# pjhusky/vulkan-compute-tests

Measured on AMD Instinct MI355X. Metric: path-traced samples/s, higher is better.
Workload: dtype f32

## Files before the change

vulkan-compute-tests_amd/csrc/mc_math.h:

```cpp
#pragma once
#include <hip/hip_runtime.h>

namespace mc {
namespace dm {

__device__ __forceinline__ float as_float(uint32_t u) { return __uint_as_float(u); }
__device__ __forceinline__ uint32_t as_uint(float f) { return __float_as_uint(f); }

__device__ __forceinline__ float ieee_div(float a, float b) { return a / b; }
__device__ __forceinline__ float ieee_sqrt(float a) { return __builtin_sqrtf(a); }

__device__ __forceinline__ bool in_short_window(float x) { return (as_uint(x) - 0x0D800000u) < 0x64000000u; }
__device__ __forceinline__ bool wave_all(bool p) { return __builtin_amdgcn_ballot_w64(!p) == 0ull; }
__device__ __forceinline__ float sqrt_short(float x) {
    float y = __builtin_amdgcn_rsqf(x);
    float g = x * y;
    float d = __builtin_fmaf(-g, g, x);
    return __builtin_fmaf(d, 0.5f * y, g);
}
__device__ __forceinline__ float rcp_short(float b) {
    float r = __builtin_amdgcn_rcpf(b);
    float e = __builtin_fmaf(-b, r, 1.0f);
    return __builtin_fmaf(e, r, r);
}

__device__ __forceinline__ float rsqrt_short(float x) {
    const float y = __builtin_amdgcn_rsqf(x);
    const float g = x * y;
    const float d = __builtin_fmaf(-g, g, x);
    const float s = __builtin_fmaf(d, 0.5f * y, g);
    const float e = __builtin_fmaf(-s, y, 1.0f);
    const float r = __builtin_fmaf(e, y, y);
    const uint32_t tie = ((as_uint(x) & 0x00fffffeu) == 0x007ffffeu) ? 1u : 0u;
    return as_float(as_uint(r) + tie);
}

__device__ __forceinline__ float div_step(float a, float s, float y) {
    const float q0 = a * y;
    const float r = __builtin_fmaf(-s, q0, a);
    return __builtin_fmaf(r, y, q0);
}

template <int Fast> __device__ __forceinline__ float fdiv(float a, float b) {
    if (Fast == 2) return div_step(a, b, rcp_short(b));
    if (Fast) return a * __builtin_amdgcn_rcpf(b);
    return ieee_div(a, b);
}
template <int Fast, bool HaveY> __device__ __forceinline__ void div3(float& a0, float& a1, float& a2, float s, float y) {
    if constexpr (!Fast) {
        const uint32_t b0 = as_uint(a0), b1 = as_uint(a1), b2 = as_uint(a2);
        uint32_t hi = b0 > b1 ? b0 : b1; hi = hi > b2 ? hi : b2;
        const uint32_t l0 = b0 - 1u, l1 = b1 - 1u, l2 = b2 - 1u;
        uint32_t lo = l0 < l1 ? l0 : l1; lo = lo < l2 ? lo : l2;
        const bool outside = ((as_uint(s) - 0x21800000u) >= 0x3C000000u) | (hi >= 0x5D800000u) | (lo < 0x21800000u - 1u);
        if constexpr (!HaveY) y = rcp_short(s);
        const float q0 = div_step(a0, s, y), q1 = div_step(a1, s, y), q2 = div_step(a2, s, y);
        if (__builtin_expect(outside, 0)) { a0 = ieee_div(a0, s); a1 = ieee_div(a1, s); a2 = ieee_div(a2, s); }
        else { a0 = q0; a1 = q1; a2 = q2; }
        return;
    }
    a0 = fdiv<Fast>(a0, s); a1 = fdiv<Fast>(a1, s); a2 = fdiv<Fast>(a2, s);
}
template <int Fast> __device__ __forceinline__ float fsqrt(float a) {
    if (Fast == 2) { const float r = sqrt_short(a); return a == 0.0f ? 0.0f : r; }
    if (Fast) return __builtin_amdgcn_sqrtf(a);
    if (__builtin_expect(wave_all(in_short_window(a)), 1)) return sqrt_short(a);
    return ieee_sqrt(a);
}
template <int Fast> __device__ __forceinline__ float inversesqrt(float a) {
    if (Fast == 2) return rsqrt_short(a);
    if (Fast) return __builtin_amdgcn_rsqf(a);
    if (__builtin_expect(wave_all(in_short_window(a)), 1)) return rsqrt_short(a);
    return ieee_div(1.0f, ieee_sqrt(a));
}

__device__ __forceinline__ void sincos_reduce(float x, float& r, int& k) {
    const float TWO_OVER_PI = 0.636619772367581343f;
    const float PIO2_HI = 1.5703125f;
    const float PIO2_MID = 4.837512969970703125e-4f;
    const float PIO2_LO = 7.54978995489188216e-8f;
    float q = __builtin_rintf(x * TWO_OVER_PI);
    r = __builtin_fmaf(q, -PIO2_HI, x);
    r = __builtin_fmaf(q, -PIO2_MID, r);
    r = __builtin_fmaf(q, -PIO2_LO, r);
    k = (int)q;
}
__device__ __forceinline__ float sin_kernel(float r) {
    float z = r * r;
    float p = __builtin_fmaf(-1.9515295891e-4f, z, 8.3321608736e-3f);
    p = __builtin_fmaf(p, z, -1.6666654611e-1f);
    return __builtin_fmaf(p * z, r, r);
}
__device__ __forceinline__ float cos_kernel(float r) {
    float z = r * r;
    float p = __builtin_fmaf(2.443315711809948e-5f, z, -1.388731625493765e-3f);
    p = __builtin_fmaf(p, z, 4.166664568298827e-2f);
    float t = __builtin_fmaf(-0.5f, z, 1.0f);
    return __builtin_fmaf(p * z, z, t);
}
__device__ __forceinline__ float mc_sin(float x) {
    float r; int k; sincos_reduce(x, r, k);
    float s = (k & 1) ? cos_kernel(r) : sin_kernel(r);
    return (k & 2) ? -s : s;
}
__device__ __forceinline__ float mc_cos(float x) {
    float r; int k; sincos_reduce(x, r, k);
    float c = (k & 1) ? sin_kernel(r) : cos_kernel(r);
    return ((k + 1) & 2) ? -c : c;
}
__device__ __forceinline__ void mc_sincos(float x, float& s, float& c) {
    float r; int k; sincos_reduce(x, r, k);
    float sk = sin_kernel(r), ck = cos_kernel(r);
    float sv = (k & 1) ? ck : sk;
    float cv = (k & 1) ? sk : ck;
    s = as_float(as_uint(sv) ^ (((uint32_t)k << 30) & 0x80000000u));
    c = as_float(as_uint(cv) ^ (((uint32_t)(k + 1) << 30) & 0x80000000u));
}

template <int Fast> __device__ __forceinline__ void sincos_angle(float angle, float u, float& s, float& c) {
    if (Fast) {
        s = __builtin_amdgcn_sinf(u);
        c = __builtin_amdgcn_cosf(u);
    } else {
        mc_sincos(angle, s, c);
    }
}

#ifdef MC_PT_TRANS_UNGROUPED
constexpr bool kTransGroups = false;
#else
constexpr bool kTransGroups = true;
#endif
__device__ __forceinline__ void light_trans_group(float xcc, float u, float& inv_len, float& s, float& c) {
    inv_len = xcc;
    asm volatile("s_setprio 3\n\t"
                 "v_rsq_f32_e32 %0, %0\n\t"
                 "v_sin_f32_e32 %1, %3\n\t"
                 "v_cos_f32_e32 %2, %3\n\t"
                 "s_setprio 0\n\t"
                 "s_nop 0"
                 : "+v"(inv_len), "=&v"(s), "=&v"(c) : "v"(u));
}
__device__ __forceinline__ void bounce_trans_group(float u1, float u2, float& r2s, float& s1, float& c1, float& C) {
    C = 1.0f - u2;
    asm volatile("s_setprio 3\n\t"
                 "v_sqrt_f32_e32 %0, %5\n\t"
                 "v_sin_f32_e32 %1, %4\n\t"
                 "v_cos_f32_e32 %2, %4\n\t"
                 "v_sqrt_f32_e32 %3, %3\n\t"
                 "s_setprio 0\n\t"
                 "s_nop 0"
                 : "=&v"(r2s), "=&v"(s1), "=&v"(c1), "+v"(C) : "v"(u1), "v"(u2));
}

__device__ __forceinline__ float mc_log2(float x) {
    if (x == 0.0f) return -__builtin_inff();
    int e_adj = 0;
    if (x < 1.17549435e-38f) { x = x * 16777216.0f; e_adj = -24; }
    uint32_t u = as_uint(x);
    int e = (int)(u >> 23) - 127;
// ... 44 lines not shown
```

vulkan-compute-tests_amd/csrc/pathtrace_kernel.h:

```cpp
#pragma once
#include <hip/hip_runtime.h>

#include <cstdlib>
#include <type_traits>
#include <utility>

#include "mc_internal.h"
#include "ds_arith.h"
#include "mc_math.h"

namespace mc {
namespace pt {

constexpr int kMaxPlanes = 16;
constexpr int kMaxSpheres = 16;
constexpr int kMaxSlabSpheres = 8;

struct v3 {
    float x, y, z;
};

struct SceneArgs {
    uint32_t n_planes, n_spheres;
    uint32_t emissive_mask;
    uint32_t nee_skip_planes;
    uint32_t materials_known;
    uint32_t emit_skip_ok;
    uint32_t box_ok;
    float obj[(kMaxPlanes + kMaxSpheres) * 12];
    float r2[kMaxSpheres];
    float slab_w_pos[3], slab_w_neg[3];
    int32_t slab_id_pos[3], slab_id_neg[3];
    const float* d_obj;
    const float* d_obj_derived;
    const uint32_t* d_emissive;
    uint32_t n_emissive;
    uint32_t spheres_disjoint;
    uint32_t pad3, pad4;
};

struct PTArgs {
    uint32_t W, H, spp, sample_begin, sample_end, max_depth, row_begin, row_end, row_block, row_stride;
    v3 cam_o, cam_d, cx, cy, lc;
    float cam_oc[kMaxSlabSpheres][3], cam_occ[kMaxSlabSpheres];
    float inv_W, inv_H, inv_spp;
    float4* __restrict__ out;
    uint32_t* status;
    SceneArgs scene;
};

__device__ __forceinline__ v3 operator+(v3 a, v3 b) { return v3{a.x + b.x, a.y + b.y, a.z + b.z}; }
__device__ __forceinline__ v3 operator-(v3 a, v3 b) { return v3{a.x - b.x, a.y - b.y, a.z - b.z}; }
__device__ __forceinline__ v3 operator*(v3 a, v3 b) { return v3{a.x * b.x, a.y * b.y, a.z * b.z}; }
__device__ __forceinline__ v3 operator*(v3 a, float s) { return v3{a.x * s, a.y * s, a.z * s}; }
__device__ __forceinline__ v3 operator-(v3 a) { return v3{-a.x, -a.y, -a.z}; }
__device__ __forceinline__ float dot(v3 a, v3 b) { return (a.x * b.x + a.y * b.y) + a.z * b.z; }
__device__ __forceinline__ v3 cross(v3 a, v3 b) {
    return v3{a.y * b.z - b.y * a.z, a.z * b.x - b.z * a.x, a.x * b.y - b.x * a.y};
}
template <int Fast> __device__ __forceinline__ v3 normalize(v3 a) { return a * dm::inversesqrt<Fast>(dot(a, a)); }
template <int Fast, bool HaveY> __device__ __forceinline__ v3 divs_impl(v3 a, float s, float y) {
    dm::div3<Fast, HaveY>(a.x, a.y, a.z, s, y);
    return a;
}
template <int Fast> __device__ __forceinline__ v3 divs(v3 a, float s) { return divs_impl<Fast, false>(a, s, 0.0f); }
template <int Fast> __device__ __forceinline__ v3 divs_recip(v3 a, float s, float y) { return divs_impl<Fast, true>(a, s, y); }
template <int Fast> __device__ __forceinline__ v3 tangent_u(v3 w) {
    const bool sel = __builtin_fabsf(w.x) > 0.1f;
    if constexpr (Fast) {
        const float q = sel ? w.x : w.y;
        const float inv = dm::inversesqrt<Fast>(__builtin_fmaf(q, q, w.z * w.z));
        const float zi = w.z * inv, qi = q * inv;
        return v3{sel ? zi : 0.0f, sel ? 0.0f : -zi, sel ? -qi : qi};
    } else {
        return normalize<false>(cross(sel ? v3{0, 1, 0} : v3{1, 0, 0}, w));
    }
}
template <int Fast, bool UnitBasis> __device__ __forceinline__ v3 normalize_unit_combination(v3 a) {
    if constexpr (Fast == 1 && UnitBasis) return a;
    else return normalize<Fast>(a);
}
__device__ __forceinline__ v3 reflect(v3 I, v3 N) { return I - N * (2.0f * dot(N, I)); }
__device__ __forceinline__ v3 select(bool c, v3 a, v3 b) { return v3{c ? a.x : b.x, c ? a.y : b.y, c ? a.z : b.z}; }
__device__ __forceinline__ float comp(v3 a, int axis) { return axis == 0 ? a.x : (axis == 1 ? a.y : a.z); }

__device__ __forceinline__ v3 rand01(uint32_t x, uint32_t y, uint32_t z) {
#pragma unroll
    for (int i = 0; i < 3; i++) {
        uint32_t nx = ((x >> 8) ^ y) * 1103515245u;
        uint32_t ny = ((y >> 8) ^ z) * 1103515245u;
        uint32_t nz = ((z >> 8) ^ x) * 1103515245u;
        x = nx; y = ny; z = nz;
    }
    const float s = 2.3283064365386963e-10f;
    return v3{(float)x * s, (float)y * s, (float)z * s};
}

#ifdef MC_PT_REGION_STATS
static __device__ unsigned long long g_region_exec[32];
static __device__ unsigned long long g_region_lanes[32];
#define MC_REGION(r)                                                                            \
    do {                                                                                        \
        unsigned long long m_ = __ballot(1);                                                    \
        if ((int)__lane_id() == __ffsll((long long)m_) - 1) {                                   \
            atomicAdd(&g_region_exec[r], 1ull);                                                 \
            atomicAdd(&g_region_lanes[r], (unsigned long long)__popcll(m_));                    \
        }                                                                                       \
    } while (0)
#define MC_PT_REGION_STATS_READER(name)                                                                              \
    int name(unsigned long long* exec32, unsigned long long* lanes32) {                                              \
        unsigned long long e[32], l[32], zero[32] = {0};                                                             \
        if (hipMemcpyFromSymbol(e, HIP_SYMBOL(mc::pt::g_region_exec), sizeof(zero)) != hipSuccess) return 3;         \
        if (hipMemcpyFromSymbol(l, HIP_SYMBOL(mc::pt::g_region_lanes), sizeof(zero)) != hipSuccess) return 3;        \
        if (hipMemcpyToSymbol(HIP_SYMBOL(mc::pt::g_region_exec), zero, sizeof(zero)) != hipSuccess) return 3;        \
        if (hipMemcpyToSymbol(HIP_SYMBOL(mc::pt::g_region_lanes), zero, sizeof(zero)) != hipSuccess) return 3;       \
        for (int i = 0; i < 32; i++) { exec32[i] += e[i]; lanes32[i] += l[i]; }                                      \
        return 0;                                                                                                    \
    }
#else
#define MC_REGION(r) do { } while (0)
#define MC_PT_REGION_STATS_READER(name)
#endif

#ifndef MC_PT_DECISION_FP
#define MC_PT_DECISION_FP
#endif

constexpr float kEps = 1e-4f, kTriEps = 1e-7f, kInf = 1e20f;
constexpr float kPi = 3.141592653589793f;
constexpr float kInvPi = 1.0f / kPi;
static_assert(kInvPi == 0x1.45f306p-2f, "1/pi must be the correctly rounded fp32 quotient (numpy: float32(1)/float32(pi) = 0x3ea2f983)");

__device__ __forceinline__ bool needs_precision(const float* sp, v3 o) {
    const float maxLen = 500.0f;
    v3 c{sp[0], sp[1], sp[2]};
    v3 co = c - o;
    return sp[3] > maxLen || dot(c, c) > maxLen * maxLen || dot(o, o) > maxLen * maxLen || dot(co, co) > maxLen * maxLen;
}
template <int Fast, int Prec>
__device__ __forceinline__ bool sphere_extended(const float* sp, float r2, v3 o, v3 d, float& dd) {
    auto rsq = [](float x) { return dm::inversesqrt<Fast>(x); };
    if (Prec == 1) {
        double ocx = (double)sp[0] - (double)o.x, ocy = (double)sp[1] - (double)o.y, ocz = (double)sp[2] - (double)o.z;
        double dx = d.x, dy = d.y, dz = d.z;
        double b = (ocx * dx + ocy * dy) + ocz * dz;
        double det = (b * b - ((ocx * ocx + ocy * ocy) + ocz * ocz)) + (double)r2;
        if (det < 0) return false;
        det = __builtin_sqrt(det);
        dd = (float)(b - det);
        if (!(dd > kEps)) { dd = (float)(b + det); if (!(dd > kEps)) dd = kInf; }
        return true;
    } else if (Prec == 2) {
        ds2 ocX = ds_add(ds_set(sp[0]), ds_set(-o.x)), ocY = ds_add(ds_set(sp[1]), ds_set(-o.y)), ocZ = ds_add(ds_set(sp[2]), ds_set(-o.z));
        ds2 rdX = ds_set(d.x), rdY = ds_set(d.y), rdZ = ds_set(d.z);
        ds2 b = ds_dot3(ocX, ocY, ocZ, rdX, rdY, rdZ);
        ds2 w = ds_set(sp[3]);
        ds2 det = ds_add(ds_sub(ds_mul(b, b), ds_dot3(ocX, ocY, ocZ, ocX, ocY, ocZ)), ds_mul(w, w));
        if (ds_compare(det, ds_set(0.0f)) < 0.0f) return false;
        det = ds_sqrt(det, rsq);
        ds2 eps_ds = ds_set(kEps);
        ds2 bMinus = ds_sub(b, det), bPlus = ds_add(b, det);
        ds2 d_ds = bMinus;
        dd = d_ds.hi;
        if (ds_compare(d_ds, eps_ds) <= 0.0f) {
            d_ds = bPlus;
            dd = d_ds.hi;
            if (ds_compare(d_ds, eps_ds) <= 0.0f) dd = kInf;
        }
        return true;
    } else {
        ds2 ocX = df64_add(df64_from_f32(sp[0]), df64_from_f32(-o.x)), ocY = df64_add(df64_from_f32(sp[1]), df64_from_f32(-o.y)),
            ocZ = df64_add(df64_from_f32(sp[2]), df64_from_f32(-o.z));
        ds2 rdX = df64_from_f32(d.x), rdY = df64_from_f32(d.y), rdZ = df64_from_f32(d.z);
        ds2 b = df64_dot3(ocX, ocY, ocZ, rdX, rdY, rdZ);
        ds2 w = df64_from_f32(sp[3]);
        ds2 det = df64_add(df64_add(df64_mult(b, b), df64_mult(df64_dot3(ocX, ocY, ocZ, ocX, ocY, ocZ), df64_from_f32(-1.0f))),
                           df64_mult(w, w));
        if (df64_lt(det, df64_from_f32(0.0f))) return false;
        det = df64_sqrt(det, rsq);
        float bMinus = df64_add(b, df64_mult(det, df64_from_f32(-1.0f))).hi;
        float bPlus = df64_add(b, det).hi;
        dd = bMinus;
        if (!(dd > kEps)) { dd = bPlus; if (!(dd > kEps)) dd = kInf; }
        return true;
    }
}

__device__ __forceinline__ float to_vgpr(float uniform) {
    float v;
    asm volatile("v_mov_b32 %0, %1" : "=v"(v) : "s"(uniform));
    return v;
}
template <int NS> struct HotSlabN {
    static constexpr int ns = NS;
    float W_pos[3], W_negm[3];
    float c[NS][3], r2[NS];
    float eps, tri_eps, inf;
    template <bool InVgpr = true, bool WPosInVgpr = false> __device__ __forceinline__ void load(const SceneArgs& sc) {
        auto put = [](float u) { return InVgpr ? to_vgpr(u) : u; };
#pragma unroll
        for (int a = 0; a < 3; a++) { W_pos[a] = (InVgpr || WPosInVgpr) ? to_vgpr(sc.slab_w_pos[a]) : sc.slab_w_pos[a]; W_negm[a] = put(-sc.slab_w_neg[a]); }
#pragma unroll
        for (int i = 0; i < NS; i++) {
#pragma unroll
            for (int k = 0; k < 3; k++) c[i][k] = put(sc.obj[12 * (6 + i) + k]);
            r2[i] = put(sc.r2[i]);
        }
        eps = put(1e-4f); tri_eps = put(1e-7f); inf = put(1e20f);
    }
};

template <int Fast, bool Closed, bool OccR2, int StatsBase, bool HaveOc, int NS>
__device__ __forceinline__ int intersect_slab_impl(const HotSlabN<NS>& h, v3 o, v3 d, float& t_out, bool shadow_skip_planes,
                                                   const float* occ,
                                                   const v3* oc_at_o) {
    MC_PT_DECISION_FP
    static_assert(HaveOc || !OccR2, "the r^2-reduced squared lengths come from the caller");
    float t = h.inf;
    int id = -1;
    if (Fast && !shadow_skip_planes) {
        float num[3], den[3];
#pragma unroll
        for (int a = 0; a < 3; a++) {
            const float da = comp(d, a), oa = comp(o, a);
            const bool pos = da > 0.0f;
            num[a] = (pos ? h.W_pos[a] : h.W_negm[a]) - oa; den[a] = da;
        }
        float bn = num[0], bd = den[0];
        int bid = 1;
#pragma unroll
        for (int a = 1; a < 3; a++) {
            const bool nearer = __builtin_fabsf(num[a]) * __builtin_fabsf(bd) < __builtin_fabsf(bn) * __builtin_fabsf(den[a]);
            bn = nearer ? num[a] : bn; bd = nearer ? den[a] : bd; bid = nearer ? 2 * a + 1 : bid;
        }
        bid ^= (int)(dm::as_uint(bd) >> 31);
        const float dd = dm::fdiv<Fast>(bn, bd);
        if constexpr (Closed) { t = dd; id = bid; }
        else if (__builtin_fabsf(bd) > h.tri_eps && dd < t) { t = dd; id = bid; }
    } else if (!shadow_skip_planes) {
#pragma unroll
        for (int a = 0; a < 3; a++) {
            const float da = comp(d, a), oa = comp(o, a);
            const bool pos = da > 0.0f;
            const float W = pos ? h.W_pos[a] : h.W_negm[a];
            const float dd = dm::fdiv<Fast>(W - oa, da);
            if (__builtin_fabsf(da) > h.tri_eps && dd < t) { t = dd; id = pos ? 2 * a + 1 : 2 * a; }
        }
    }
#pragma unroll
    for (int i = 0; i < NS; i++) {
        v3 oc;
        if constexpr (HaveOc) oc = oc_at_o[i]; else oc = v3{h.c[i][0], h.c[i][1], h.c[i][2]} - o;
        float b = dot(oc, d);
        float occ_i;
        if constexpr (HaveOc) occ_i = occ[i]; else occ_i = dot(oc, oc);
        float det = OccR2 ? b * b - occ_i : (b * b - occ_i) + h.r2[i];
        if (!(det < 0.0f)) {
            if constexpr (StatsBase >= 0) MC_REGION(StatsBase + i);
            float sq = dm::fsqrt<Fast>(det);
            float dd = b - sq;
            if (dd <= h.eps) {
                dd = b + sq;
                if (dd <= h.eps) dd = h.inf;
            }
            if (dd < t) { t = dd; id = 6 + i; }
        }
    }
    t_out = t;
    if constexpr (Closed) return id;
    return (t < h.inf) ? id : -1;
}
template <int Fast, bool Closed = false, bool OccR2 = false, int StatsBase = -1, int NS = 3>
__device__ __forceinline__ int intersect_slab(const HotSlabN<NS>& h, v3 o, v3 d, float& t_out, bool shadow_skip_planes) {
    return intersect_slab_impl<Fast, Closed, OccR2, StatsBase, false, NS>(h, o, d, t_out, shadow_skip_planes, nullptr, nullptr);
}
template <int Fast, bool Closed = false, bool OccR2 = false, int StatsBase = -1, int NS = 3>
__device__ __forceinline__ int intersect_slab(const HotSlabN<NS>& h, v3 o, v3 d, float& t_out, bool shadow_skip_planes,
                                              const float* occ, const v3* oc_at_o) {
    return intersect_slab_impl<Fast, Closed, OccR2, StatsBase, true, NS>(h, o, d, t_out, shadow_skip_planes, occ, oc_at_o);
}

template <int Fast, bool OccR2 = false, int NS = 3>
__device__ __forceinline__ bool shadow_reaches_sphere(const HotSlabN<NS>& h, v3 o, v3 d, int li, v3 oc_li, const float* occ) {
    MC_PT_DECISION_FP
    float dd[NS];
#pragma unroll
    for (int i = 0; i < NS; i++) {
        const v3 oc = i == li ? oc_li : v3{h.c[i][0], h.c[i][1], h.c[i][2]} - o;
        float b = dot(oc, d);
        float det = OccR2 ? b * b - occ[i] : (b * b - occ[i]) + h.r2[i];
        float r = h.inf;
        if (!(det < 0.0f)) {
            float sq = dm::fsqrt<Fast>(det);
            r = b - sq;
            if (r <= h.eps) {
                r = b + sq;
                if (r <= h.eps) r = h.inf;
            }
        }
        dd[i] = r;
    }
    bool nearest = true;
#pragma unroll
    for (int k = 0; k < NS; k++) {
        if (k < li) nearest = nearest && dd[li] < dd[k];
        else if (k > li) nearest = nearest && !(dd[k] < dd[li]);
    }
    if (Fast && li == NS - 1 && NS > 1) return nearest;
    return nearest && dd[li] < h.inf;
}

template <bool OccR2, int NS>
__device__ __forceinline__ bool shadow_visible_disjoint(const HotSlabN<NS>& h, v3 d, int li, const v3* xoc, const float* occ) {
    MC_PT_DECISION_FP
    float b[NS];
    bool hit[NS];
#pragma unroll
    for (int i = 0; i < NS; i++) {
        b[i] = dot(xoc[i], d);
        const float det = OccR2 ? b[i] * b[i] - occ[i] : (b[i] * b[i] - occ[i]) + h.r2[i];
        if (i == li) { hit[i] = det >= 0.0f; continue; }
        const float e = b[i] - h.eps;
        hit[i] = !(det < 0.0f) && (e > 0.0f || det > e * e);
    }
    bool vis = hit[li];
#pragma unroll
    for (int i = 0; i < NS; i++)
        if (i != li) vis = vis && !(hit[i] && b[i] < b[li]);
    return vis;
}


template <int Fast, int NP, int NS, bool Slab, int Prec>
__device__ __forceinline__ int intersect(const SceneArgs& sc, const float* __restrict__ obj, v3 o, v3 d, float& t_out,
                                         bool shadow_skip_planes = false) {
    MC_PT_DECISION_FP
    constexpr bool LdsScene = NP < 0;
    const int np = NP >= 0 ? NP : (int)sc.n_planes;
    const int ns = NS >= 0 ? NS : (int)sc.n_spheres;
    float t = kInf;
    int id = -1;
    if (Slab && shadow_skip_planes) {
    } else if (Slab) {
#pragma unroll
        for (int a = 0; a < 3; a++) {
            const float da = comp(d, a), oa = comp(o, a);
            const bool pos = da > 0.0f;
            const float den = __builtin_fabsf(da);
            const float num = pos ? (sc.slab_w_pos[a] - oa) : (sc.slab_w_neg[a] + oa);
            const float dd = dm::fdiv<Fast>(num, den);
            if (den > kTriEps && dd < t) { t = dd; id = pos ? 2 * a + 1 : 2 * a; }
        }
    } else {
#pragma unroll
// ... 483 lines not shown
```

vulkan-compute-tests_amd/csrc/pathtrace_pool.h:

```cpp
#pragma once
#include <type_traits>
#include "pathtrace_kernel.h"

namespace mc {
namespace pt {

#ifdef MC_PT_POOL_PARENT_FORMS
constexpr bool kPoolParentForms = true;
#else
constexpr bool kPoolParentForms = false;
#endif
#if defined(MC_PT_POOL_FLOAT_STATE) || defined(MC_PT_POOL_PARENT_FORMS)
constexpr bool kPoolFloatState = true;
#else
constexpr bool kPoolFloatState = false;
#endif
__device__ __forceinline__ unsigned long long lanes_where(bool cmp) { return __builtin_amdgcn_ballot_w64(cmp); }
__device__ __forceinline__ bool lane_in(unsigned long long m) { return __builtin_amdgcn_inverse_ballot_w64(m); }
__device__ __forceinline__ v3 add_emission(v3 rad, v3 accmat, v3 e) {
#pragma clang fp contract(off)
    const float px = accmat.x * e.x, py = accmat.y * e.y, pz = accmat.z * e.z;
    return v3{rad.x + px, rad.y + py, rad.z + pz};
}
constexpr uint32_t kPoolEntryFloats = 8;
constexpr uint32_t kPoolRecordStride = 16;
template <int NS> constexpr uint32_t pool_record_floats() { return (6u + (uint32_t)NS) * kPoolRecordStride; }
constexpr uint32_t kPoolStashFloats = 128u * kPoolEntryFloats;
template <int NS> constexpr uint32_t pool_result_batches() { return NS <= 3 ? 3u : 4u; }
template <int NS> constexpr uint32_t pool_result_floats() { return 64u * pool_result_batches<NS>() * 3u; }
template <int Fast, int NS> constexpr uint32_t pool_wave_lds_floats() { return kPoolStashFloats + (Fast ? 0u : pool_result_floats<NS>()); }
template <int Fast, int NS> constexpr size_t pool_block_lds_bytes() { return (pool_record_floats<NS>() + 4u * pool_wave_lds_floats<Fast, NS>()) * sizeof(float); }
template <int Fast, int NS> constexpr int pool_waves() {
    constexpr int kFast3 = 7;
    constexpr int kStrict3 = 6;
    return Fast ? (NS <= 3 ? kFast3 : NS <= 5 ? 6 : NS <= 6 ? 5 : 4) : (NS <= 3 ? kStrict3 : NS <= 6 ? 4 : 3);
}

template <int Fast, int NS> constexpr bool pool_parent_state() { return kPoolFloatState || (Fast == 1 && NS == 2); }
template <int Fast, int NS> constexpr bool pool_lane_masks() { return !pool_parent_state<Fast, NS>() && Fast != 0 && !(Fast == 2 && NS == 7); }
template <int Fast, int NS> constexpr bool pool_emis_cond() { return !pool_parent_state<Fast, NS>(); }

template <int Fast, int S, int NS, bool Disjoint = true>
__global__ void __launch_bounds__(256, (pool_waves<Fast, NS>())) pathtrace_pool_kernel(PTArgs a) {
    constexpr uint32_t kPoolRecordFloats = pool_record_floats<NS>();
    extern __shared__ float lds_dyn[];
    float* lds_obj = lds_dyn;
    if (threadIdx.x < 6u + (uint32_t)NS) {
        const float* o = a.scene.obj + 12u * threadIdx.x;
        float* r = lds_obj + kPoolRecordStride * threadIdx.x;
        const float p = dm::gmax(dm::gmax(o[8], o[9]), o[10]);
        r[0] = o[0]; r[1] = o[1]; r[2] = o[2]; r[3] = Fast ? dm::fdiv<Fast>(1.0f, p) : p;
        r[4] = o[8]; r[5] = o[9]; r[6] = o[10];
        const uint32_t emits = (o[4] != 0.0f || o[5] != 0.0f || o[6] != 0.0f) ? 256u : 0u;
        r[7] = dm::as_float((uint32_t)(int)__builtin_floorf(o[11] + 0.5f) | emits);
        r[8] = o[4]; r[9] = o[5]; r[10] = o[6]; r[11] = Fast ? p : dm::rcp_short(p);
        if constexpr (Fast) { r[12] = o[8] * r[3]; r[13] = o[9] * r[3]; r[14] = o[10] * r[3]; r[15] = r[7]; }
    }
    __syncthreads();
    constexpr bool kOccR2 = Fast == 1;
    constexpr bool kLaneMasks = pool_lane_masks<Fast, NS>(), kEmisCond = pool_emis_cond<Fast, NS>(), kOneAlpha = kEmisCond;
    constexpr bool kGrouped = Fast == 1 && dm::kTransGroups;
    constexpr uint32_t TW = WaveTile<S>::w, TH = WaveTile<S>::h, Ring = 2u * (uint32_t)S, RRing = pool_result_batches<NS>() * (uint32_t)S;
    HotSlabN<NS> hot;
    hot.template load<false, true>(a.scene);
    struct Lane { uint32_t lane, pix, sub, ty; bool valid; };
    auto my_lane = [&](bool with_row) {
        uint32_t tid = threadIdx.x;
        if (Fast == 0 || with_row) asm volatile("" : "+v"(tid));
        Lane q;
        q.lane = tid & 63u; q.pix = q.lane / (uint32_t)S; q.sub = q.lane % (uint32_t)S;
        const uint32_t wave = tid >> 6;
        q.ty = 0u; q.valid = false;
        if (with_row) {
            q.ty = blockIdx.y * (2u * TH) + (wave >> 1) * TH + q.pix / TW;
            const uint32_t gxx = blockIdx.x * (2u * TW) + (wave & 1u) * TW + q.pix % TW;
            q.valid = gxx < a.W && tile_row_to_storage(q.ty, a.row_begin, a.row_block, a.row_stride) < a.row_end;
        }
        return q;
    };
    uint32_t gx, gy;
    bool pixel_valid;
    float* const gstash = lds_dyn + kPoolRecordFloats + (threadIdx.x >> 6) * pool_wave_lds_floats<Fast, NS>() +
                          ((threadIdx.x & 63u) / (uint32_t)S) * (Ring * kPoolEntryFloats);
    float* const gres = lds_dyn + kPoolRecordFloats + (threadIdx.x >> 6) * pool_wave_lds_floats<Fast, NS>() + kPoolStashFloats +
                        ((threadIdx.x & 63u) / (uint32_t)S) * (3u * RRing);
    {
        const uint32_t tid = threadIdx.x, wave = tid >> 6, pix = (tid & 63u) / (uint32_t)S;
        gx = blockIdx.x * (2u * TW) + (wave & 1u) * TW + pix % TW;
        const uint32_t ty = blockIdx.y * (2u * TH) + (wave >> 1) * TH + pix / TW;
        const uint32_t srow = tile_row_to_storage(ty, a.row_begin, a.row_block, a.row_stride);
        pixel_valid = gx < a.W && srow < a.row_end;
        gy = a.H - 1u - (pixel_valid ? srow : 0u);
    }
    const uint32_t n_batches = (a.sample_end - a.sample_begin + (uint32_t)S - 1u) / (uint32_t)S;
    uint32_t batch = 0u;
    uint32_t ghead = 0u;
    v3 ro{0, 0, 0}, rd{0, 0, 1}, accmat{1, 1, 1}, acc{0, 0, 0};
    v3 accrad{0, 0, 0};
    if constexpr (!Fast) {
        if (a.sample_begin > 0u) {
            const Lane me = my_lane(true);
            if (me.valid) { const float4 prev = a.out[(size_t)me.ty * a.W + gx]; acc = v3{prev.x, prev.y, prev.z}; }
        }
    }
    uint32_t cur = 0u;
    uint32_t committed = 0u;
    const float fspp = __int_as_float(__builtin_amdgcn_readfirstlane(__float_as_int((float)a.spp)));
    float emissive = 1.0f, t = 0.0f, occ[NS];
#pragma unroll
    for (int i = 0; i < NS; i++) occ[i] = 0.0f;
    int id = 0;
    uint32_t key = 0u, kend = 0u, krr = 0u;
    float rx = 0.0f, ry = 0.0f;
    bool alive = false;
    unsigned long long alive_m = 0ull;
    bool emis = true;
    unsigned long long max_iters = (unsigned long long)n_batches * S * (a.max_depth + 2ull) + 64ull;
#ifdef MC_PT_POOL_TEST_BOUND
    max_iters = MC_PT_POOL_TEST_BOUND;
#endif
    bool finished = false;
    for (unsigned long long it = 0; it < max_iters; it++) {
        MC_REGION(0);
        const unsigned long long deadm = kLaneMasks ? ~alive_m & lanes_where(true) : __ballot(!alive);
        if (deadm != 0ull) {
            MC_REGION(1);
            const Lane me = my_lane(false);
            const uint32_t gbits = (uint32_t)(deadm >> (me.lane - me.sub)) & (S == 32 ? ~0u : ((1u << (S & 31)) - 1u));
            const uint32_t need = (uint32_t)__builtin_popcount(gbits);
            uint32_t avail = batch * (uint32_t)S - ghead;
            bool want = batch < n_batches && __ballot(need > avail) != 0ull && __ballot(avail > (uint32_t)S) == 0ull;
            if constexpr (!Fast) {
                if (want) {
                    uint32_t oldest = alive ? cur : 0xffffffffu;
                    if constexpr (S == 16) {
                        auto rot_min = [](uint32_t v, auto ctrl) {
                            const uint32_t o = (uint32_t)__builtin_amdgcn_update_dpp((int)v, (int)v, decltype(ctrl)::value, 0xf, 0xf, false);
                            return o < v ? o : v;
                        };
                        oldest = rot_min(oldest, std::integral_constant<int, 0x128>{});
                        oldest = rot_min(oldest, std::integral_constant<int, 0x124>{});
                        oldest = rot_min(oldest, std::integral_constant<int, 0x122>{});
                        oldest = rot_min(oldest, std::integral_constant<int, 0x121>{});
                    } else {
#pragma unroll
                        for (uint32_t o = 1; o < (uint32_t)S; o <<= 1) {
                            const uint32_t other = (uint32_t)__builtin_amdgcn_ds_bpermute((int)((me.lane ^ o) << 2), (int)oldest);
                            oldest = other < oldest ? other : oldest;
                        }
                    }
                    const uint32_t fin = oldest < ghead ? oldest : ghead;
                    while (committed + (uint32_t)S <= fin) {
                        for (uint32_t k = 0; k < (uint32_t)S; k++) {
                            const uint32_t slot = (committed + k) % RRing;
                            acc.x += gres[slot]; acc.y += gres[RRing + slot]; acc.z += gres[2u * RRing + slot];
                        }
                        committed += (uint32_t)S;
                    }
                    want = __ballot((batch + 1u) * (uint32_t)S - committed > RRing) == 0ull;
                }
            }
            if (want) {
                MC_REGION(2);
                const Lane g = my_lane(false);
                const uint32_t samp = a.sample_begin + batch * (uint32_t)S + g.sub;
                uint32_t cgx = gx, cgy = gy;
                if constexpr (!Fast) asm volatile("" : "+v"(cgx), "+v"(cgy));
                const v3 crd = camera_ray<Fast>(a, cgx, cgy, samp);
                v3 oc0[NS];
                float occ0[NS], ct;
#pragma unroll
                for (int i = 0; i < NS; i++) {
                    oc0[i] = v3{a.cam_oc[i][0], a.cam_oc[i][1], a.cam_oc[i][2]};
                    occ0[i] = kOccR2 ? a.cam_occ[i] - hot.r2[i] : a.cam_occ[i];
                }
                int cid = intersect_slab<Fast, (Fast != 0), kOccR2, 22>(hot, a.lc, crd, ct, false, occ0, oc0);
                if (!(pixel_valid && samp < a.sample_end)) cid = -1;
                if constexpr (!Fast) {
                    const uint32_t slot = (batch * (uint32_t)S + g.sub) % RRing;
                    if (cid < 0) { gres[slot] = 0.0f; gres[RRing + slot] = 0.0f; gres[2u * RRing + slot] = 0.0f; }
                }
                float4* e = reinterpret_cast<float4*>(gstash + ((batch * (uint32_t)S + g.sub) & (Ring - 1u)) * kPoolEntryFloats);
                e[0] = make_float4(crd.x, crd.y, crd.z, ct);
                const v3 r0 = rand01(gx, gy, samp * a.max_depth);
                e[1] = make_float4(dm::as_float((uint32_t)cid), dm::as_float(samp * a.max_depth), r0.x, r0.y);
                batch++;
                avail += (uint32_t)S;
            }
            const uint32_t rank = (uint32_t)__builtin_popcount(gbits & ((1u << me.sub) - 1u));
            const unsigned long long take_m = kLaneMasks ? deadm & lanes_where(rank < avail) : 0ull;
            if (kLaneMasks ? lane_in(take_m) : (!alive && rank < avail)) {
                MC_REGION(3);
                const float4* q = reinterpret_cast<const float4*>(gstash + ((ghead + rank) & (Ring - 1u)) * kPoolEntryFloats);
                const float4 q0 = q[0], q1 = q[1];
                rd = v3{q0.x, q0.y, q0.z}; t = q0.w;
                if constexpr (!Fast) { cur = ghead + rank; accrad = v3{0.0f, 0.0f, 0.0f}; }
                id = (int)dm::as_uint(q1.x);
                key = dm::as_uint(q1.y); kend = key + a.max_depth; krr = key + 5u;
                rx = q1.z; ry = q1.w;
                ro = a.lc;
                accmat = v3{1.0f, 1.0f, 1.0f};
                if constexpr (kEmisCond) emis = true; else emissive = 1.0f;
                if constexpr (!kLaneMasks) alive = id >= 0;
            }
            if constexpr (kLaneMasks) alive_m |= take_m & lanes_where(id >= 0);
            ghead += need < avail ? need : avail;
        }
#ifdef MC_PT_POOL_PARENT_FORMS
        if (__ballot(alive) == 0ull && batch >= n_batches && __ballot(ghead != batch * (uint32_t)S) == 0ull) { finished = true; break; }
#else
        if (batch >= n_batches && (kLaneMasks ? alive_m : __ballot(alive)) == 0ull && __ballot(ghead != batch * (uint32_t)S) == 0ull) { finished = true; break; }
#endif
        v3 xoc[NS];
        if (kLaneMasks ? lane_in(alive_m) : alive) {
            {
                MC_REGION(4);
                unsigned long long sph_m = 0ull;
                if constexpr (!kPoolParentForms) sph_m = __ballot(id >= 6);
                v3 x = ro + rd * t;
#pragma unroll
                for (int i = 0; i < NS; i++) { xoc[i] = v3{hot.c[i][0], hot.c[i][1], hot.c[i][2]} - x; occ[i] = dot(xoc[i], xoc[i]); }
                float xcc[NS];
#pragma unroll
                for (int i = 0; i < NS; i++) { xcc[i] = occ[i]; if constexpr (kOccR2) occ[i] = occ[i] - hot.r2[i]; }
                const float4* obj = reinterpret_cast<const float4*>(lds_obj + kPoolRecordStride * (uint32_t)id);
                const float4 o0 = obj[0], o1 = obj[(Fast && key > krr) ? 3 : 1];
                const bool is_sphere = id >= 6;
                v3 geo{o0.x, o0.y, o0.z};
                v3 col{o1.x, o1.y, o1.z};
                const uint32_t mbits = dm::as_uint(o1.w);
                const int mat = (int)(mbits & 255u);
#ifdef MC_PT_REGION_STATS
                if (is_sphere) MC_REGION(5);
#endif
                v3 n = is_sphere ? normalize<Fast>(x - geo) : geo;
                const float dot_n_rd = dot(n, rd);
                v3 nl;
                if constexpr (Fast) {
                    const uint32_t flip = ~dm::as_uint(dot_n_rd) & 0x80000000u;
                    nl = v3{dm::as_float(dm::as_uint(n.x) ^ flip), dm::as_float(dm::as_uint(n.y) ^ flip), dm::as_float(dm::as_uint(n.z) ^ flip)};
                } else {
                    nl = dot_n_rd < 0.0f ? n : -n;
                }
                v3& rad = Fast ? acc : accrad;
                if constexpr (!kEmisCond) {
                if (__ballot(mbits >= 256u) != 0ull) {
                    MC_REGION(12);
                    const float4 o2 = obj[2];
                    rad = rad + (accmat * v3{o2.x, o2.y, o2.z}) * emissive;
                }
                } else if (mbits >= 256u && emis) {
                    MC_REGION(12);
                    const float4 o2 = obj[2];
                    rad = add_emission(rad, accmat, v3{o2.x, o2.y, o2.z});
                }
                accmat = accmat * col;
                const v3 rnd{rx, ry, 0.0f};
                if constexpr (!Fast) { if (key > krr) accmat = divs_recip<Fast>(accmat, o0.w, obj[2].w); }
                bool go = true;
                {
                ro = x;
                if (mat == 1) {
                    MC_REGION(13);
                    v3 accmat_over_pi{0.0f, 0.0f, 0.0f};
                    if constexpr (!Fast) accmat_over_pi = divs_recip<Fast>(accmat, kPi, kInvPi);
#pragma unroll
                    for (int i = 0; i < NS; i++) {
                        if (!((a.scene.emissive_mask >> i) & 1u)) continue;
                        const float* ls = a.scene.obj + 12 * (6 + i);
                        v3 le{ls[4], ls[5], ls[6]};
                        float cos_a_max;
                        v3 l = light_sample_direction<Fast, kGrouped>(xoc[i], xcc[i], hot.r2[i], rnd, cos_a_max);
                        bool lit;
                        if constexpr (Fast && Disjoint) lit = shadow_visible_disjoint<kOccR2>(hot, l, i, xoc, occ);
                        else lit = shadow_reaches_sphere<Fast, kOccR2>(hot, x, l, i, xoc[i], occ);
                        if (lit) {
                            MC_REGION(8);
                            if constexpr (Fast) {
                                const float scale = __builtin_fmaxf(dot(l, nl), 0.0f) * (2.0f - (cos_a_max + cos_a_max));
                                rad = rad + (accmat * le) * scale;
                            } else {
                                const float omega = (2.0f * kPi) * (1.0f - cos_a_max);
                                rad = rad + ((accmat_over_pi * dm::gmax(dot(l, nl), 0.0f)) * le) * omega;
                            }
                        }
                    }
                    auto walls_only = [&]() {
                        if constexpr (kPoolParentForms) return __ballot(is_sphere) == 0ull;
                        else return (sph_m & __ballot(true)) == 0ull;
                    };
                    if constexpr (kGrouped) {
                        const BounceTrans bt = bounce_trans_grouped(rnd);
                        if (walls_only()) { MC_REGION(9); rd = cosine_bounce_wall_grouped(id, bt); }
                        else { MC_REGION(10); rd = cosine_bounce_grouped<true>(nl, bt); }
                    } else if (walls_only()) { MC_REGION(9); rd = cosine_bounce_wall<Fast>(id, rnd); }
                    else { MC_REGION(10); rd = cosine_bounce<Fast, true>(nl, rnd); }
                    if constexpr (kEmisCond) emis = false; else emissive = 0.0f;
                } else {
                    MC_REGION(11);
                    if constexpr (Fast) rd = specular_bounce_fast<Fast, kOneAlpha>(mat, rd, n, dot_n_rd, rnd.x, accmat);
                    else rd = specular_bounce_general<false, true>(mat, rd, n, nl, dot_n_rd, rnd.x, accmat);
                    if constexpr (kEmisCond) emis = true; else emissive = 1.0f;
                }
                if constexpr (!kLaneMasks) {
                key++;
                go = key != kend;
                if (go) {
                    MC_REGION(14);
                    id = intersect_slab<Fast, (Fast != 0), kOccR2, 16>(hot, ro, rd, t, false, occ, xoc);
                    go = id >= 0;
                }
                if (go) {
                    const v3 rn = rand01(gx, gy, key);
                    rx = rn.x; ry = rn.y;
                    if (key > krr) {
                        MC_REGION(15);
                        const float4* nobj = reinterpret_cast<const float4*>(lds_obj + kPoolRecordStride * (uint32_t)id);
                        go = !(rn.z >= nobj[Fast ? 2 : 0].w);
                        if constexpr (kPoolParentForms) {
                            if (__ballot(!go && dm::as_uint(nobj[1].w) >= 256u) != 0ull) {
                                const float4 o2 = nobj[2];
                                if (!go) rad = rad + (accmat * v3{o2.x, o2.y, o2.z}) * emissive;
                            }
                        } else if constexpr (kEmisCond) {
                            if (!go && dm::as_uint(nobj[1].w) >= 256u && emis) {
                                const float4 o2 = nobj[2];
                                rad = add_emission(rad, accmat, v3{o2.x, o2.y, o2.z});
                            }
                        } else if (!go && dm::as_uint(nobj[1].w) >= 256u) {
                            const float4 o2 = nobj[2];
                            rad = rad + (accmat * v3{o2.x, o2.y, o2.z}) * emissive;
                        }
                    }
                }
                }
                }
                if constexpr (!Fast && !kLaneMasks) {
                    if (!go) {
                        const v3 q = divs_recip<Fast>(accrad, fspp, a.inv_spp);
                        const uint32_t slot = cur % RRing;
                        gres[slot] = q.x; gres[RRing + slot] = q.y; gres[2u * RRing + slot] = q.z;
                    }
                }
                if constexpr (!kLaneMasks) alive = go;
            }
        }
        if constexpr (kLaneMasks) {
            static_assert(Fast != 0 || !kLaneMasks, "the strict kernels keep `alive` per lane: the mask form spilled (pool_lane_masks)");
            v3& rad = acc;
            key++;
            alive_m &= lanes_where(key != kend);
            if (lane_in(alive_m)) {
                MC_REGION(14);
                id = intersect_slab<Fast, (Fast != 0), kOccR2, 16>(hot, ro, rd, t, false, occ, xoc);
            }
            const v3 rn = rand01(gx, gy, key);
            rx = rn.x; ry = rn.y;
            const unsigned long long deep_m = alive_m & lanes_where(key > krr);
            const float4* nobj = reinterpret_cast<const float4*>(lds_obj + kPoolRecordStride * (uint32_t)id);
            float pn;
            asm volatile("" : "=v"(pn));
            if (lane_in(deep_m)) {
                MC_REGION(15);
                pn = nobj[2].w;
            }
            const unsigned long long end_m = deep_m & lanes_where(rn.z >= pn);
            alive_m &= ~end_m;
            if (lane_in(end_m)) {
                if (dm::as_uint(nobj[1].w) >= 256u && emis) {
                    const float4 o2 = nobj[2];
                    rad = add_emission(rad, accmat, v3{o2.x, o2.y, o2.z});
                }
            }
        }
    }
    if (!finished && a.status && (threadIdx.x & 63u) == 0u) atomicOr(a.status, 2u);
    float4 sum = make_float4(0.0f, 0.0f, 0.0f, 0.0f);
    const Lane fin = my_lane(true);
    if constexpr (Fast) {
        auto from_lane = [](float v, uint32_t src) {
            return __int_as_float(__builtin_amdgcn_ds_bpermute((int)(src << 2), __float_as_int(v)));
        };
        for (uint32_t k = 0; k < (uint32_t)S; k++) {
            const uint32_t src = fin.lane - fin.sub + k;
            sum.x += from_lane(acc.x, src); sum.y += from_lane(acc.y, src); sum.z += from_lane(acc.z, src);
        }
        sum.x *= a.inv_spp; sum.y *= a.inv_spp; sum.z *= a.inv_spp;
        if (a.sample_begin > 0u && fin.valid) {
            const float4 prev = a.out[(size_t)fin.ty * a.W + gx];
            sum.x += prev.x; sum.y += prev.y; sum.z += prev.z;
        }
    } else {
        while (committed < n_batches * (uint32_t)S) {
            for (uint32_t k = 0; k < (uint32_t)S; k++) {
                const uint32_t slot = (committed + k) % RRing;
                acc.x += gres[slot]; acc.y += gres[RRing + slot]; acc.z += gres[2u * RRing + slot];
            }
            committed += (uint32_t)S;
        }
        sum = make_float4(acc.x, acc.y, acc.z, 0.0f);
    }
    if (a.sample_end == a.spp) {
        sum.x = dm::fpow<Fast>(dm::gmin(dm::gmax(sum.x, 0.0f), 1.0f), 0.45f) * 255.0f + 0.5f;
        sum.y = dm::fpow<Fast>(dm::gmin(dm::gmax(sum.y, 0.0f), 1.0f), 0.45f) * 255.0f + 0.5f;
        sum.z = dm::fpow<Fast>(dm::gmin(dm::gmax(sum.z, 0.0f), 1.0f), 0.45f) * 255.0f + 0.5f;
    }
    if (fin.valid && fin.sub == 0u) a.out[(size_t)fin.ty * a.W + gx] = sum;
}

template <int Fast, int S, int NS> inline int launch_pool_one(const PTArgs& a, uint32_t tile_rows, hipStream_t s) {
    dim3 grid((a.W + block_w<S>() - 1u) / block_w<S>(), (tile_rows + block_h<S>() - 1u) / block_h<S>());
    constexpr size_t lds = pool_block_lds_bytes<Fast, NS>();
    if (Fast && !a.scene.spheres_disjoint) hipLaunchKernelGGL((pathtrace_pool_kernel<Fast, S, NS, false>), grid, dim3(256), lds, s, a);
    else hipLaunchKernelGGL((pathtrace_pool_kernel<Fast, S, NS, true>), grid, dim3(256), lds, s, a);
    return MC_OK;
}
template <int Fast> inline int launch_pool(const PTArgs& a, int S, uint32_t tile_rows, hipStream_t s) {
    if (S != 16) return MC_ERR_INVALID_ARGUMENT;
    return dispatch_spheres(a.scene.n_spheres, [&](auto NS) { return launch_pool_one<Fast, 16, NS>(a, tile_rows, s); });
}

template <int Fast> int launch_tier(const PTArgs& a, int kernel, int S, int prec, uint32_t tile_rows, hipStream_t s) {
    if (kernel == MC_PT_KERNEL_POOL) return launch_pool<Fast>(a, S, tile_rows, s);
    if (prec != 0)
        return dispatch<1, 2, 3>(prec, [&](auto P) {
            return dispatch<1, 16>(S, [&](auto W) { return launch_one<Fast, -1, -1, false, W, P>(a, tile_rows, s); });
        });
    switch (kernel) {
        case MC_PT_KERNEL_BOX:
            if constexpr (Fast != 0) return launch_slab<Fast, true>(a, S, tile_rows, s);
            return MC_ERR_INVALID_ARGUMENT;
        case MC_PT_KERNEL_SLAB: return launch_slab<Fast, false>(a, S, tile_rows, s);
        case MC_PT_KERNEL_GENERIC_MEMORY:
            return dispatch<1, 4, 16>(S, [&](auto W) { return launch_one<Fast, -2, -2, false, W, 0>(a, tile_rows, s); });
        default: return dispatch<1, 4, 16>(S, [&](auto W) { return launch_one<Fast, -1, -1, false, W, 0>(a, tile_rows, s); });
    }
}

}
}
```

Measured before the change: 20.38 billion.

## Trim per-bounce ALU and registers in pool kernel fast tiers

Adds a bundle of micro-optimizations for the fast pool kernel variants. It stores the emission flag apart from the material code, and scales the Russian-roulette threshold by 2^32 so the random z needs no scaling. It also folds the normal flip into a bitop3 applied to the dot product, carries the deep-row mask across iterations, and skips per-lane hit checks for full batches of valid pixels. These changes aim to cut VALU instructions and register pressure on the hot bounce loop. In exchange they add layout and semantic coupling between record fields, and the new conditions can break if scene assumptions change.

```diff
diff --git a/vulkan-compute-tests_amd/csrc/mc_math.h b/vulkan-compute-tests_amd/csrc/mc_math.h
--- a/vulkan-compute-tests_amd/csrc/mc_math.h
+++ b/vulkan-compute-tests_amd/csrc/mc_math.h
@@ -6,6 +6,19 @@
 
 __device__ __forceinline__ float as_float(uint32_t u) { return __uint_as_float(u); }
 __device__ __forceinline__ uint32_t as_uint(float f) { return __float_as_uint(f); }
+__device__ __forceinline__ float flip_where_sign_clear(float v, float s) {
+#if defined(__HIP_DEVICE_COMPILE__)
+    return as_float(__builtin_amdgcn_bitop3_b32(as_uint(s), as_uint(v), 0x80000000u, 0xc6));
+#else
+    return as_float(as_uint(v) ^ (~as_uint(s) & 0x80000000u));
+#endif
+}
+
+__device__ __forceinline__ float max_zero_as_is(float v) {
+    float r;
+    asm("v_max_f32_e32 %0, 0, %1" : "=v"(r) : "v"(v));
+    return r;
+}
 
 __device__ __forceinline__ float ieee_div(float a, float b) { return a / b; }
 __device__ __forceinline__ float ieee_sqrt(float a) { return __builtin_sqrtf(a); }
diff --git a/vulkan-compute-tests_amd/csrc/pathtrace_kernel.h b/vulkan-compute-tests_amd/csrc/pathtrace_kernel.h
--- a/vulkan-compute-tests_amd/csrc/pathtrace_kernel.h
+++ b/vulkan-compute-tests_amd/csrc/pathtrace_kernel.h
@@ -84,7 +84,7 @@
 __device__ __forceinline__ v3 select(bool c, v3 a, v3 b) { return v3{c ? a.x : b.x, c ? a.y : b.y, c ? a.z : b.z}; }
 __device__ __forceinline__ float comp(v3 a, int axis) { return axis == 0 ? a.x : (axis == 1 ? a.y : a.z); }
 
-__device__ __forceinline__ v3 rand01(uint32_t x, uint32_t y, uint32_t z) {
+__device__ __forceinline__ v3 rand_hash_unscaled(uint32_t x, uint32_t y, uint32_t z) {
 #pragma unroll
     for (int i = 0; i < 3; i++) {
         uint32_t nx = ((x >> 8) ^ y) * 1103515245u;
@@ -92,8 +92,16 @@
         uint32_t nz = ((z >> 8) ^ x) * 1103515245u;
         x = nx; y = ny; z = nz;
     }
-    const float s = 2.3283064365386963e-10f;
-    return v3{(float)x * s, (float)y * s, (float)z * s};
+    return v3{(float)x, (float)y, (float)z};
+}
+constexpr float kRandScale = 2.3283064365386963e-10f;
+__device__ __forceinline__ v3 rand01(uint32_t x, uint32_t y, uint32_t z) {
+    const v3 h = rand_hash_unscaled(x, y, z);
+    return v3{h.x * kRandScale, h.y * kRandScale, h.z * kRandScale};
+}
+__device__ __forceinline__ v3 rand01_zraw(uint32_t x, uint32_t y, uint32_t z) {
+    const v3 h = rand_hash_unscaled(x, y, z);
+    return v3{h.x * kRandScale, h.y * kRandScale, h.z};
 }
 
 #ifdef MC_PT_REGION_STATS
@@ -196,10 +204,13 @@
     float W_pos[3], W_negm[3];
     float c[NS][3], r2[NS];
     float eps, tri_eps, inf;
-    template <bool InVgpr = true, bool WPosInVgpr = false> __device__ __forceinline__ void load(const SceneArgs& sc) {
+    template <bool InVgpr = true, bool WPosInVgpr = false, int WNegInVgpr = 0> __device__ __forceinline__ void load(const SceneArgs& sc) {
         auto put = [](float u) { return InVgpr ? to_vgpr(u) : u; };
 #pragma unroll
-        for (int a = 0; a < 3; a++) { W_pos[a] = (InVgpr || WPosInVgpr) ? to_vgpr(sc.slab_w_pos[a]) : sc.slab_w_pos[a]; W_negm[a] = put(-sc.slab_w_neg[a]); }
+        for (int a = 0; a < 3; a++) {
+            W_pos[a] = (InVgpr || WPosInVgpr) ? to_vgpr(sc.slab_w_pos[a]) : sc.slab_w_pos[a];
+            W_negm[a] = (InVgpr || a < WNegInVgpr) ? to_vgpr(-sc.slab_w_neg[a]) : -sc.slab_w_neg[a];
+        }
 #pragma unroll
         for (int i = 0; i < NS; i++) {
 #pragma unroll
diff --git a/vulkan-compute-tests_amd/csrc/pathtrace_pool.h b/vulkan-compute-tests_amd/csrc/pathtrace_pool.h
--- a/vulkan-compute-tests_amd/csrc/pathtrace_pool.h
+++ b/vulkan-compute-tests_amd/csrc/pathtrace_pool.h
@@ -21,6 +21,9 @@
 #pragma clang fp contract(off)
     const float px = accmat.x * e.x, py = accmat.y * e.y, pz = accmat.z * e.z;
     return v3{rad.x + px, rad.y + py, rad.z + pz};
+}
+__device__ __forceinline__ v3 nl_of(v3 n, float dot_n_rd) {
+    return v3{dm::flip_where_sign_clear(n.x, dot_n_rd), dm::flip_where_sign_clear(n.y, dot_n_rd), dm::flip_where_sign_clear(n.z, dot_n_rd)};
 }
 constexpr uint32_t kPoolEntryFloats = 8;
 constexpr uint32_t kPoolRecordStride = 16;
@@ -40,6 +43,19 @@
 template <int Fast, int NS> constexpr bool pool_lane_masks() { return !pool_parent_state<Fast, NS>() && Fast != 0 && !(Fast == 2 && NS == 7); }
 template <int Fast, int NS> constexpr bool pool_emis_cond() { return !pool_parent_state<Fast, NS>(); }
 
+#if defined(MC_PT_POOL_DIET3_PARENT) || defined(MC_PT_POOL_FLOAT_STATE) || defined(MC_PT_POOL_PARENT_FORMS)
+constexpr bool kPoolDiet3Parent = true;
+#else
+constexpr bool kPoolDiet3Parent = false;
+#endif
+template <int Fast, int NS> constexpr bool pool_diet3() { return !kPoolDiet3Parent && !pool_parent_state<Fast, NS>() && !(Fast != 0 && NS == 8); }
+template <int Fast, int NS> constexpr bool pool_deep_carry() { return pool_diet3<Fast, NS>() && pool_lane_masks<Fast, NS>(); }
+template <int Fast, int NS> constexpr bool pool_nl_dot() { return pool_diet3<Fast, NS>() && Fast != 0; }
+template <int Fast, int NS> constexpr int pool_wneg_vgprs() { return pool_diet3<Fast, NS>() && Fast != 0 ? 3 : 0; }
+template <int Fast, int NS> constexpr bool pool_rr_unscaled() { return pool_diet3<Fast, NS>() && Fast != 0; }
+template <int Fast, int NS> constexpr bool pool_live_entries() { return pool_diet3<Fast, NS>() && pool_lane_masks<Fast, NS>(); }
+template <int Fast, int NS> constexpr bool pool_flag_apart() { return pool_diet3<Fast, NS>() && Fast != 0; }
+
 template <int Fast, int S, int NS, bool Disjoint = true>
 __global__ void __launch_bounds__(256, (pool_waves<Fast, NS>())) pathtrace_pool_kernel(PTArgs a) {
     constexpr uint32_t kPoolRecordFloats = pool_record_floats<NS>();
@@ -49,20 +65,26 @@
         const float* o = a.scene.obj + 12u * threadIdx.x;
         float* r = lds_obj + kPoolRecordStride * threadIdx.x;
         const float p = dm::gmax(dm::gmax(o[8], o[9]), o[10]);
-        r[0] = o[0]; r[1] = o[1]; r[2] = o[2]; r[3] = Fast ? dm::fdiv<Fast>(1.0f, p) : p;
+        const float r3 = Fast ? dm::fdiv<Fast>(1.0f, p) : p;
+        r[0] = o[0]; r[1] = o[1]; r[2] = o[2]; r[3] = r3;
         r[4] = o[8]; r[5] = o[9]; r[6] = o[10];
         const uint32_t emits = (o[4] != 0.0f || o[5] != 0.0f || o[6] != 0.0f) ? 256u : 0u;
-        r[7] = dm::as_float((uint32_t)(int)__builtin_floorf(o[11] + 0.5f) | emits);
-        r[8] = o[4]; r[9] = o[5]; r[10] = o[6]; r[11] = Fast ? p : dm::rcp_short(p);
-        if constexpr (Fast) { r[12] = o[8] * r[3]; r[13] = o[9] * r[3]; r[14] = o[10] * r[3]; r[15] = r[7]; }
+        constexpr bool kFlagApart = pool_flag_apart<Fast, NS>();
+        const uint32_t mcode = (uint32_t)(int)__builtin_floorf(o[11] + 0.5f);
+        r[7] = dm::as_float(kFlagApart ? mcode : (mcode | emits));
+        r[8] = o[4]; r[9] = o[5]; r[10] = o[6]; r[11] = Fast ? (pool_rr_unscaled<Fast, NS>() ? p * 4294967296.0f : p) : dm::rcp_short(p);
+        if constexpr (Fast) { r[12] = o[8] * r3; r[13] = o[9] * r3; r[14] = o[10] * r3; r[15] = r[7]; }
+        if constexpr (kFlagApart) r[3] = dm::as_float(emits);
     }
     __syncthreads();
     constexpr bool kOccR2 = Fast == 1;
     constexpr bool kLaneMasks = pool_lane_masks<Fast, NS>(), kEmisCond = pool_emis_cond<Fast, NS>(), kOneAlpha = kEmisCond;
     constexpr bool kGrouped = Fast == 1 && dm::kTransGroups;
+    constexpr bool kDeepCarry = pool_deep_carry<Fast, NS>(), kNlDot = pool_nl_dot<Fast, NS>(), kRrUnscaled = pool_rr_unscaled<Fast, NS>(),
+                   kLiveEntries = pool_live_entries<Fast, NS>(), kFlagApart = pool_flag_apart<Fast, NS>();
     constexpr uint32_t TW = WaveTile<S>::w, TH = WaveTile<S>::h, Ring = 2u * (uint32_t)S, RRing = pool_result_batches<NS>() * (uint32_t)S;
     HotSlabN<NS> hot;
-    hot.template load<false, true>(a.scene);
+    hot.template load<false, true, pool_wneg_vgprs<Fast, NS>()>(a.scene);
     struct Lane { uint32_t lane, pix, sub, ty; bool valid; };
     auto my_lane = [&](bool with_row) {
         uint32_t tid = threadIdx.x;
@@ -115,6 +137,13 @@
     bool alive = false;
     unsigned long long alive_m = 0ull;
     bool emis = true;
+    unsigned long long deep_row_m = 0ull;
+    bool pixels_live = false;
+    uint32_t full_batches = 0u;
+    if constexpr (kLiveEntries) {
+        pixels_live = __ballot(!pixel_valid) == 0ull;
+        full_batches = (a.sample_end - a.sample_begin) % (uint32_t)S == 0u ? n_batches : n_batches - 1u;
+    }
     unsigned long long max_iters = (unsigned long long)n_batches * S * (a.max_depth + 2ull) + 64ull;
 #ifdef MC_PT_POOL_TEST_BOUND
     max_iters = MC_PT_POOL_TEST_BOUND;
@@ -203,7 +232,10 @@
                 if constexpr (kEmisCond) emis = true; else emissive = 1.0f;
                 if constexpr (!kLaneMasks) alive = id >= 0;
             }
-            if constexpr (kLaneMasks) alive_m |= take_m & lanes_where(id >= 0);
+            if constexpr (kLiveEntries) {
+                if (pixels_live && batch <= full_batches) alive_m |= take_m;
+                else alive_m |= take_m & lanes_where(id >= 0);
+            } else if constexpr (kLaneMasks) alive_m |= take_m & lanes_where(id >= 0);
             ghead += need < avail ? need : avail;
         }
 #ifdef MC_PT_POOL_PARENT_FORMS
@@ -224,19 +256,24 @@
 #pragma unroll
                 for (int i = 0; i < NS; i++) { xcc[i] = occ[i]; if constexpr (kOccR2) occ[i] = occ[i] - hot.r2[i]; }
                 const float4* obj = reinterpret_cast<const float4*>(lds_obj + kPoolRecordStride * (uint32_t)id);
-                const float4 o0 = obj[0], o1 = obj[(Fast && key > krr) ? 3 : 1];
+                const bool deep_row = kDeepCarry ? lane_in(deep_row_m) : (Fast && key > krr);
+                const float4 o0 = obj[0], o1 = obj[deep_row ? 3 : 1];
                 const bool is_sphere = id >= 6;
                 v3 geo{o0.x, o0.y, o0.z};
                 v3 col{o1.x, o1.y, o1.z};
                 const uint32_t mbits = dm::as_uint(o1.w);
-                const int mat = (int)(mbits & 255u);
+                const int mat = kFlagApart ? (int)mbits : (int)(mbits & 255u);
+                const bool hit_emits = kFlagApart ? dm::as_uint(o0.w) != 0u : mbits >= 256u;
 #ifdef MC_PT_REGION_STATS
                 if (is_sphere) MC_REGION(5);
 #endif
                 v3 n = is_sphere ? normalize<Fast>(x - geo) : geo;
                 const float dot_n_rd = dot(n, rd);
                 v3 nl;
-                if constexpr (Fast) {
+                if constexpr (kNlDot) {
+                    static_assert(!kNlDot || Fast != 0, "the flipped dot product is the fast and careful tiers' form: strict reads nl");
+                    nl = n;
+                } else if constexpr (Fast) {
                     const uint32_t flip = ~dm::as_uint(dot_n_rd) & 0x80000000u;
                     nl = v3{dm::as_float(dm::as_uint(n.x) ^ flip), dm::as_float(dm::as_uint(n.y) ^ flip), dm::as_float(dm::as_uint(n.z) ^ flip)};
                 } else {
@@ -249,7 +286,7 @@
                     const float4 o2 = obj[2];
                     rad = rad + (accmat * v3{o2.x, o2.y, o2.z}) * emissive;
                 }
-                } else if (mbits >= 256u && emis) {
+                } else if (hit_emits && emis) {
                     MC_REGION(12);
                     const float4 o2 = obj[2];
                     rad = add_emission(rad, accmat, v3{o2.x, o2.y, o2.z});
@@ -277,7 +314,9 @@
                         if (lit) {
                             MC_REGION(8);
                             if constexpr (Fast) {
-                                const float scale = __builtin_fmaxf(dot(l, nl), 0.0f) * (2.0f - (cos_a_max + cos_a_max));
+                                const float l_nl = kNlDot ? dm::flip_where_sign_clear(dot(l, n), dot_n_rd) : dot(l, nl);
+                                const float cosine = kNlDot ? dm::max_zero_as_is(l_nl) : __builtin_fmaxf(l_nl, 0.0f);
+                                const float scale = cosine * (2.0f - (cos_a_max + cos_a_max));
                                 rad = rad + (accmat * le) * scale;
                             } else {
                                 const float omega = (2.0f * kPi) * (1.0f - cos_a_max);
@@ -292,9 +331,9 @@
                     if constexpr (kGrouped) {
                         const BounceTrans bt = bounce_trans_grouped(rnd);
                         if (walls_only()) { MC_REGION(9); rd = cosine_bounce_wall_grouped(id, bt); }
-                        else { MC_REGION(10); rd = cosine_bounce_grouped<true>(nl, bt); }
+                        else { MC_REGION(10); rd = cosine_bounce_grouped<true>(kNlDot ? nl_of(n, dot_n_rd) : nl, bt); }
                     } else if (walls_only()) { MC_REGION(9); rd = cosine_bounce_wall<Fast>(id, rnd); }
-                    else { MC_REGION(10); rd = cosine_bounce<Fast, true>(nl, rnd); }
+                    else { MC_REGION(10); rd = cosine_bounce<Fast, true>(kNlDot ? nl_of(n, dot_n_rd) : nl, rnd); }
                     if constexpr (kEmisCond) emis = false; else emissive = 0.0f;
                 } else {
                     MC_REGION(11);
@@ -311,7 +350,7 @@
                     go = id >= 0;
                 }
                 if (go) {
-                    const v3 rn = rand01(gx, gy, key);
+                    const v3 rn = kRrUnscaled ? rand01_zraw(gx, gy, key) : rand01(gx, gy, key);
                     rx = rn.x; ry = rn.y;
                     if (key > krr) {
                         MC_REGION(15);
@@ -323,7 +362,7 @@
                                 if (!go) rad = rad + (accmat * v3{o2.x, o2.y, o2.z}) * emissive;
                             }
                         } else if constexpr (kEmisCond) {
-                            if (!go && dm::as_uint(nobj[1].w) >= 256u && emis) {
+                            if (!go && (kFlagApart ? dm::as_uint(nobj[0].w) != 0u : dm::as_uint(nobj[1].w) >= 256u) && emis) {
                                 const float4 o2 = nobj[2];
                                 rad = add_emission(rad, accmat, v3{o2.x, o2.y, o2.z});
                             }
@@ -354,7 +393,7 @@
                 MC_REGION(14);
                 id = intersect_slab<Fast, (Fast != 0), kOccR2, 16>(hot, ro, rd, t, false, occ, xoc);
             }
-            const v3 rn = rand01(gx, gy, key);
+            const v3 rn = kRrUnscaled ? rand01_zraw(gx, gy, key) : rand01(gx, gy, key);
             rx = rn.x; ry = rn.y;
             const unsigned long long deep_m = alive_m & lanes_where(key > krr);
             const float4* nobj = reinterpret_cast<const float4*>(lds_obj + kPoolRecordStride * (uint32_t)id);
@@ -366,8 +405,9 @@
             }
             const unsigned long long end_m = deep_m & lanes_where(rn.z >= pn);
             alive_m &= ~end_m;
+            if constexpr (kDeepCarry) deep_row_m = deep_m & ~end_m;
             if (lane_in(end_m)) {
-                if (dm::as_uint(nobj[1].w) >= 256u && emis) {
+                if ((kFlagApart ? dm::as_uint(nobj[0].w) != 0u : dm::as_uint(nobj[1].w) >= 256u) && emis) {
                     const float4 o2 = nobj[2];
                     rad = add_emission(rad, accmat, v3{o2.x, o2.y, o2.z});
                 }
```

New measurement: 20.72 billion, median of 6. 1.02x the previous value.
